# zhanxw/rvtests

Hardware: AMD Instinct MI355X
Metric: gene-sets/sec (SKAT+SKAT-O+CMC+Zeggini, analytic p-values) (higher is better)
Workload: dtype f64

## Files before the change

rvtests_amd/csrc/suffstat_hc.hip.h:

```cpp
#pragma once
#include <type_traits>
#include "suffstat_kernels.hip.h"

namespace rvt {

typedef int i4_t __attribute__((ext_vector_type(4)));
typedef unsigned int u4_t __attribute__((ext_vector_type(4)));

constexpr int kHcMaxMT = 6;
constexpr int kHcMaxD = 13;
constexpr int kHcStepUnit = 12;
constexpr int kHcMaxSteps = 1020;
constexpr int kHcColstatRows = 6;

constexpr int hc_pq_tiles(int MT) { return MT * MT + MT * (MT + 1) / 2; }
constexpr int hc_pq_words(int MT) { return hc_pq_tiles(MT) * 128; }
constexpr int hc_lds_words(int MT) { return hc_pq_words(MT) + 64 * MT + 4; }

struct NullTile {
  const double* base;
  int cols;
};

__device__ __forceinline__ unsigned row16_sum(unsigned h) {
  h += (unsigned)__builtin_amdgcn_update_dpp(0, (int)h, 0xB1, 0xF, 0xF, true);
  h += (unsigned)__builtin_amdgcn_update_dpp(0, (int)h, 0x4E, 0xF, 0xF, true);
  h += (unsigned)__builtin_amdgcn_update_dpp(0, (int)h, 0x141, 0xF, 0xF, true);
  h += (unsigned)__builtin_amdgcn_update_dpp(0, (int)h, 0x140, 0xF, 0xF, true);
  return h;
}

template <int MT>
struct HcStep {
  u4_t glo[MT], ghi[MT];
  u4_t xlo, xhi;
};

template <int MT, bool NT>
__device__ __forceinline__ void hc_issue(HcStep<MT>& f, const __amdgpu_buffer_rsrc_t& rg, const unsigned (&voff)[MT],
                                         const __amdgpu_buffer_rsrc_t& rx, unsigned xoff, int imm) {
#pragma unroll
  for (int c = 0; c < MT; ++c) {
    f.glo[c] = __builtin_bit_cast(u4_t, __builtin_amdgcn_raw_buffer_load_b128(rg, voff[c] + imm, 0, NT ? 2 : 0));
    f.ghi[c] = __builtin_bit_cast(u4_t, __builtin_amdgcn_raw_buffer_load_b128(rg, voff[c] + imm + 16, 0, NT ? 2 : 0));
  }
  f.xlo = __builtin_bit_cast(u4_t, __builtin_amdgcn_raw_buffer_load_b128(rx, xoff + imm, 0, 0));
  f.xhi = __builtin_bit_cast(u4_t, __builtin_amdgcn_raw_buffer_load_b128(rx, xoff + imm + 16, 0, 0));
}

__device__ __forceinline__ double hc_dbl(unsigned lo, unsigned hi) {
  return __builtin_bit_cast(double, ((unsigned long long)hi << 32) | lo);
}

struct HcBurden {
  double a_cmc, a_zeg;
  unsigned zz, cnt;
};

template <bool MASKED>
__device__ __forceinline__ void hc_row(const u4_t& glo, const u4_t& ghi, const double (&xv)[4], d4_t& accT,
                                       unsigned& pk, unsigned& mk, unsigned& cs, unsigned fx, unsigned& h, bool valid) {
  const double g0 = hc_dbl(glo[0], glo[1]), g1 = hc_dbl(glo[2], glo[3]), g2 = hc_dbl(ghi[0], ghi[1]),
               g3 = hc_dbl(ghi[2], ghi[3]);
  accT = __builtin_amdgcn_mfma_f64_16x16x4f64(g0, xv[0], accT, 0, 0, 0);
  accT = __builtin_amdgcn_mfma_f64_16x16x4f64(g1, xv[1], accT, 0, 0, 0);
  accT = __builtin_amdgcn_mfma_f64_16x16x4f64(g2, xv[2], accT, 0, 0, 0);
  accT = __builtin_amdgcn_mfma_f64_16x16x4f64(g3, xv[3], accT, 0, 0, 0);
  const unsigned w01 = __builtin_amdgcn_perm(glo[3], glo[1], 0x0c0c0703u);
  const unsigned w23 = __builtin_amdgcn_perm(ghi[3], ghi[1], 0x07030c0cu);
  unsigned p = ((w01 | w23) >> 5) & 0x03030303u;
  constexpr unsigned kAdd = 0x00100000u, kBits = 0xBFEFFFFFu;
  const unsigned i0 = ((glo[1] + kAdd) & kBits) | glo[0], i1 = ((glo[3] + kAdd) & kBits) | glo[2],
                 i2 = ((ghi[1] + kAdd) & kBits) | ghi[0], i3 = ((ghi[3] + kAdd) & kBits) | ghi[2];
  auto one = [](unsigned x) { return x < 1u ? x : 1u; };
  unsigned m = one(i0) | (one(i1) << 8) | (one(i2) << 16) | (one(i3) << 24);
  if (MASKED) {
    p = valid ? p : 0u;
    m = valid ? m : 0u;
  }
  const unsigned m3 = m * 3u;
  p &= ~m3;
  pk = p;
  mk = m;
  cs = __builtin_amdgcn_sad_u8(p, 0u, cs);
  const unsigned t = (p ^ fx) & ~m3;
  h += (t | (t >> 1)) & 0x01010101u;
}
__device__ __forceinline__ unsigned hc_code3(unsigned p) { return p & (p >> 1) & 0x01010101u; }

__device__ __forceinline__ void hc_note_masked(const u4_t& glo, const u4_t& ghi, unsigned mk, unsigned* oa) {
  auto note = [&](unsigned lo, unsigned hi) {
    __hip_atomic_fetch_or(oa + 0, lo, __ATOMIC_RELAXED, __HIP_MEMORY_SCOPE_WORKGROUP);
    __hip_atomic_fetch_or(oa + 1, hi, __ATOMIC_RELAXED, __HIP_MEMORY_SCOPE_WORKGROUP);
    __hip_atomic_fetch_and(oa + 2, lo, __ATOMIC_RELAXED, __HIP_MEMORY_SCOPE_WORKGROUP);
    __hip_atomic_fetch_and(oa + 3, hi, __ATOMIC_RELAXED, __HIP_MEMORY_SCOPE_WORKGROUP);
  };
  if (mk & 0x000000ffu) note(glo[0], glo[1]);
  if (mk & 0x0000ff00u) note(glo[2], glo[3]);
  if (mk & 0x00ff0000u) note(ghi[0], ghi[1]);
  if (mk & 0xff000000u) note(ghi[2], ghi[3]);
}

template <bool MASKED>
__device__ __forceinline__ void hc_finish(unsigned h, const double (&xv)[4], HcBurden& bu, unsigned vmask) {
  h = row16_sum(h);
  if (MASKED) h &= vmask;
#pragma unroll
  for (int l = 0; l < 4; ++l) {
    const unsigned cz = (h >> (8 * l)) & 0xffu;
    const unsigned cc = cz ? 1u : 0u;
    bu.zz = cz * cz + bu.zz;
    bu.cnt += cc;
    bu.a_zeg = fma((double)cz, xv[l], bu.a_zeg);
    bu.a_cmc = fma((double)cc, xv[l], bu.a_cmc);
  }
}

struct HcMaskCtx {
  unsigned* oa;
  unsigned* flag;
};

template <int MT, bool MASKED>
__device__ __forceinline__ void hc_step(const HcStep<MT>& f, const int T, d4_t (&accT)[MT], unsigned (&pk)[MT][4],
                                        unsigned (&cs)[MT], const unsigned (&fx)[MT], HcBurden& bu, bool valid,
                                        unsigned vmask, unsigned& anym, const HcMaskCtx& mc) {
  double xv[4] = {hc_dbl(f.xlo[0], f.xlo[1]), hc_dbl(f.xlo[2], f.xlo[3]), hc_dbl(f.xhi[0], f.xhi[1]),
                  hc_dbl(f.xhi[2], f.xhi[3])};
  if (MASKED) {
#pragma unroll
    for (int l = 0; l < 4; ++l) xv[l] = valid ? xv[l] : 0.0;
  }
  unsigned h = 0;
#pragma unroll
  for (int c = 0; c < MT; ++c) {
    unsigned p, m;
    hc_row<MASKED>(f.glo[c], f.ghi[c], xv, accT[c], p, m, cs[c], fx[c], h, valid);
    if (m) hc_note_masked(f.glo[c], f.ghi[c], m, mc.oa + 64 * c);
    if (hc_code3(p)) __hip_atomic_fetch_or(mc.flag, 2u, __ATOMIC_RELAXED, __HIP_MEMORY_SCOPE_WORKGROUP);
    pk[c][T] = p | (m << 2);
    anym |= m;
  }
  hc_finish<MASKED>(h, xv, bu, vmask);
}

template <int MT>
__device__ __forceinline__ void hc_gram(const unsigned (&pk)[MT][4], i4_t (&accS)[MT * (MT + 1) / 2]) {
  i4_t op[MT];
#pragma unroll
  for (int c = 0; c < MT; ++c) op[c] = i4_t{(int)pk[c][0], (int)pk[c][1], (int)pk[c][2], (int)pk[c][3]};
  int t = 0;
#pragma unroll
  for (int r = 0; r < MT; ++r)
#pragma unroll
    for (int c = r; c < MT; ++c, ++t) accS[t] = __builtin_amdgcn_mfma_i32_16x16x64_i8(op[r], op[c], accS[t], 0, 0, 0);
}

template <int MT>
__device__ __forceinline__ void hc_gram_masked(const unsigned (&pk)[MT][4], unsigned* lds, int lane) {
  auto mask_op = [&](int c) {
    return i4_t{(int)((pk[c][0] >> 2) & 0x01010101u), (int)((pk[c][1] >> 2) & 0x01010101u),
                (int)((pk[c][2] >> 2) & 0x01010101u), (int)((pk[c][3] >> 2) & 0x01010101u)};
  };
  auto add = [&](int tile, const i4_t& z) {
    const unsigned w0 = (unsigned)z[0] | ((unsigned)z[1] << 16), w1 = (unsigned)z[2] | ((unsigned)z[3] << 16);
    __hip_atomic_fetch_add(lds + (tile * 2 + 0) * 64 + lane, w0, __ATOMIC_RELAXED, __HIP_MEMORY_SCOPE_WORKGROUP);
    __hip_atomic_fetch_add(lds + (tile * 2 + 1) * 64 + lane, w1, __ATOMIC_RELAXED, __HIP_MEMORY_SCOPE_WORKGROUP);
  };
#pragma unroll
  for (int c = 0; c < MT; ++c) {
    const i4_t mc = mask_op(c);
#pragma unroll
    for (int r = 0; r < MT; ++r) {
      const i4_t a = i4_t{(int)pk[r][0], (int)pk[r][1], (int)pk[r][2], (int)pk[r][3]};
      add(r * MT + c, __builtin_amdgcn_mfma_i32_16x16x64_i8(a, mc, i4_t{0, 0, 0, 0}, 0, 0, 0));
      if (r <= c) {
        const i4_t mr = (r == c) ? mc : mask_op(r);
        add(MT * MT + r * MT - r * (r - 1) / 2 + (c - r), __builtin_amdgcn_mfma_i32_16x16x64_i8(mr, mc, i4_t{0, 0, 0, 0}, 0, 0, 0));
      }
    }
    __builtin_amdgcn_sched_barrier(0);
  }
  __hip_atomic_fetch_or(lds + hc_pq_words(MT) + 64 * MT, 1u, __ATOMIC_RELAXED, __HIP_MEMORY_SCOPE_WORKGROUP);
}

template <int MT>
__device__ __forceinline__ void hc_group_end(const unsigned (&pk)[MT][4], i4_t (&accS)[MT * (MT + 1) / 2], unsigned& anym,
                                             unsigned* lds, int lane) {
  hc_gram<MT>(pk, accS);
  if (__builtin_amdgcn_ballot_w64(anym != 0u) != 0ull) hc_gram_masked<MT>(pk, lds, lane);
  anym = 0u;
}

template <int MT, int DEPTH, bool NT>
__device__ __forceinline__ void suffstat_hc_body(const GeneDesc& gd, const NullTile& nt, long long N, long long ld,
                                                 int d, unsigned* lds) {
  const int lane = threadIdx.x & 63;
  const int v = lane & 15, q = lane >> 4;
  const int wpart = blockIdx.x;
  if (wpart >= gd.n_wparts) return;
  constexpr int kPQ = hc_pq_words(MT);
#pragma unroll 4
  for (int w = lane; w < kPQ; w += 64) lds[w] = 0u;
#pragma unroll
  for (int c = 0; c < MT; ++c) lds[kPQ + 64 * c + lane] = (lane & 2) ? 0xffffffffu : 0u;
  if (lane < 4) lds[kPQ + 64 * MT + lane] = 0u;
  const HcMaskCtx mc{lds + kPQ + 4 * v, lds + kPQ + 64 * MT};
  unsigned anym = 0u;
  const long long nsteps = ld >> 4;
  const long long s_begin = (long long)wpart * gd.steps_per_wpart;
  long long s_end = s_begin + gd.steps_per_wpart;
  if (s_end > nsteps) s_end = nsteps;
  if (s_begin >= s_end) return;
  const int M = gd.M;
  auto uniform = [](const void* p) {
    const unsigned long long a = (unsigned long long)p;
    const unsigned lo = __builtin_amdgcn_readfirstlane((unsigned)a);
    const unsigned hi = __builtin_amdgcn_readfirstlane((unsigned)(a >> 32));
    return (void*)(((unsigned long long)hi << 32) | lo);
  };
  const unsigned gbytes = (unsigned)((unsigned long long)M * (unsigned long long)ld * 8ull);
  const __amdgpu_buffer_rsrc_t rg = __builtin_amdgcn_make_buffer_rsrc(uniform(gd.G), 0, gbytes, 0x00020000);
  const unsigned xbytes = (unsigned)((unsigned long long)(d + 1) * (unsigned long long)ld * 8ull);
  const __amdgpu_buffer_rsrc_t rx = __builtin_amdgcn_make_buffer_rsrc(uniform(nt.base), 0, xbytes, 0x00020000);
  const unsigned lane_off = (unsigned)(q * 32);
  const unsigned col_bytes = (unsigned)((unsigned long long)ld * 8ull);
  unsigned vbase[MT];
#pragma unroll
  for (int c = 0; c < MT; ++c) {
    const int col = c * 16 + v;
    vbase[c] = (col < M) ? (unsigned)col * col_bytes + lane_off : 0x80000000u;
  }
  const unsigned xbase = (v <= d) ? (unsigned)v * col_bytes + lane_off : 0x80000000u;
  unsigned fx[MT];
#pragma unroll
  for (int c = 0; c < MT; ++c) fx[c] = ((gd.pflip[c] >> v) & 1) ? 0x02020202u : 0u;

  d4_t accT[MT];
  i4_t accS[MT * (MT + 1) / 2];
  unsigned cs[MT], pk[MT][4];
#pragma unroll
  for (int c = 0; c < MT; ++c) {
    accT[c] = d4_t{0.0, 0.0, 0.0, 0.0};
    cs[c] = 0;
  }
#pragma unroll
  for (int t = 0; t < MT * (MT + 1) / 2; ++t) accS[t] = i4_t{0, 0, 0, 0};
  HcBurden bu{0.0, 0.0, 0u, 0u};

  long long s = s_begin;
  const long long full = N >> 4;
  const long long s_fast_end = (s_end < full) ? s_end : full;
  constexpr int U = (DEPTH == 3) ? 12 : 4;
  const long long n_fast = (s_fast_end > s_begin) ? (s_fast_end - s_begin) / U : 0;
  if constexpr (DEPTH == 1) {
   if (n_fast > 0) {
    unsigned voff[MT];
#pragma unroll
    for (int c = 0; c < MT; ++c) voff[c] = vbase[c] + (unsigned)(s_begin * 128);
    unsigned xoff = xbase + (unsigned)(s_begin * 128);
    u4_t glo[MT], ghi[MT], xlo[2], xhi[2];
#pragma unroll
    for (int c = 0; c < MT; ++c) {
      glo[c] = __builtin_bit_cast(u4_t, __builtin_amdgcn_raw_buffer_load_b128(rg, voff[c], 0, NT ? 2 : 0));
      ghi[c] = __builtin_bit_cast(u4_t, __builtin_amdgcn_raw_buffer_load_b128(rg, voff[c] + 16, 0, NT ? 2 : 0));
    }
    xlo[0] = __builtin_bit_cast(u4_t, __builtin_amdgcn_raw_buffer_load_b128(rx, xoff, 0, 0));
    xhi[0] = __builtin_bit_cast(u4_t, __builtin_amdgcn_raw_buffer_load_b128(rx, xoff + 16, 0, 0));
    for (long long it = 0; it < n_fast; ++it) {
#pragma unroll
      for (int u = 0; u < 4; ++u) {
        xlo[(u + 1) & 1] = __builtin_bit_cast(u4_t, __builtin_amdgcn_raw_buffer_load_b128(rx, xoff + (u + 1) * 128, 0, 0));
        xhi[(u + 1) & 1] = __builtin_bit_cast(u4_t, __builtin_amdgcn_raw_buffer_load_b128(rx, xoff + (u + 1) * 128 + 16, 0, 0));
        __builtin_amdgcn_sched_barrier(0);
        const double xv[4] = {hc_dbl(xlo[u & 1][0], xlo[u & 1][1]), hc_dbl(xlo[u & 1][2], xlo[u & 1][3]),
                              hc_dbl(xhi[u & 1][0], xhi[u & 1][1]), hc_dbl(xhi[u & 1][2], xhi[u & 1][3])};
        unsigned h = 0;
#pragma unroll
        for (int c = 0; c < MT; ++c) {
          unsigned p, m;
          hc_row<false>(glo[c], ghi[c], xv, accT[c], p, m, cs[c], fx[c], h, true);
          if (m) hc_note_masked(glo[c], ghi[c], m, mc.oa + 64 * c);
          if (hc_code3(p)) __hip_atomic_fetch_or(mc.flag, 2u, __ATOMIC_RELAXED, __HIP_MEMORY_SCOPE_WORKGROUP);
          pk[c][u] = p | (m << 2);
          anym |= m;
          glo[c] = __builtin_bit_cast(u4_t, __builtin_amdgcn_raw_buffer_load_b128(rg, voff[c] + (u + 1) * 128, 0, NT ? 2 : 0));
          ghi[c] = __builtin_bit_cast(u4_t, __builtin_amdgcn_raw_buffer_load_b128(rg, voff[c] + (u + 1) * 128 + 16, 0, NT ? 2 : 0));
          __builtin_amdgcn_sched_barrier(0);
        }
        hc_finish<false>(h, xv, bu, 0xffffffffu);
        if (u == 3) hc_group_end<MT>(pk, accS, anym, lds, lane);
        __builtin_amdgcn_sched_barrier(0);
      }
#pragma unroll
      for (int c = 0; c < MT; ++c) voff[c] += 4 * 128;
      xoff += 4 * 128;
    }
    s += n_fast * U;
   }
  } else if (n_fast > 0) {
    unsigned voff[MT];
#pragma unroll
    for (int c = 0; c < MT; ++c) voff[c] = vbase[c] + (unsigned)(s_begin * 128);
    unsigned xoff = xbase + (unsigned)(s_begin * 128);
    HcStep<MT> f[DEPTH];
#pragma unroll
    for (int u = 0; u < DEPTH - 1; ++u) hc_issue<MT, NT>(f[u], rg, voff, rx, xoff, u * 128);
    for (long long it = 0; it < n_fast; ++it) {
#pragma unroll
      for (int u = 0; u < U; ++u) {
        hc_issue<MT, NT>(f[(u + DEPTH - 1) % DEPTH], rg, voff, rx, xoff, (u + DEPTH - 1) * 128);
        __builtin_amdgcn_sched_barrier(0);
        hc_step<MT, false>(f[u % DEPTH], u & 3, accT, pk, cs, fx, bu, true, 0xffffffffu, anym, mc);
        if ((u & 3) == 3) hc_group_end<MT>(pk, accS, anym, lds, lane);
        __builtin_amdgcn_sched_barrier(0);
      }
#pragma unroll
      for (int c = 0; c < MT; ++c) voff[c] += U * 128;
      xoff += U * 128;
    }
    s += n_fast * U;
  }
  while (s < s_end) {
#pragma unroll
    for (int c = 0; c < MT; ++c) pk[c][0] = pk[c][1] = pk[c][2] = pk[c][3] = 0u;
    auto one = [&](const int T, long long su) {
      const bool valid = su < s_end;
      const long long sc = valid ? su : s_end - 1;
      unsigned voff[MT];
#pragma unroll
      for (int c = 0; c < MT; ++c) voff[c] = vbase[c] + (unsigned)(sc * 128);
      HcStep<MT> f;
      hc_issue<MT, false>(f, rg, voff, rx, xbase + (unsigned)(sc * 128), 0);
      unsigned vmask = 0u;
      const long long smp = sc * 16 + q * 4;
#pragma unroll
      for (int l = 0; l < 4; ++l) vmask |= (valid && smp + l < N) ? (0xffu << (8 * l)) : 0u;
      hc_step<MT, true>(f, T, accT, pk, cs, fx, bu, valid, vmask, anym, mc);
    };
    one(0, s);
    one(1, s + 1);
    one(2, s + 2);
    one(3, s + 3);
    hc_group_end<MT>(pk, accS, anym, lds, lane);
    s += 4;
  }

  double* out = gd.parts + (long long)wpart * gd.Mp * gd.Cp;
  const int Cp = gd.Cp;
  {
    int t = 0;
#pragma unroll
    for (int r = 0; r < MT; ++r)
#pragma unroll
      for (int c = r; c < MT; ++c, ++t) {
        const int col = c * 16 + v;
        if (col < M) {
#pragma unroll
          for (int i = 0; i < 4; ++i) out[(long long)(r * 16 + q * 4 + i) * Cp + col] = (double)accS[t][i];
        }
      }
  }
#pragma unroll
  for (int r = 0; r < MT; ++r) {
#pragma unroll
    for (int i = 0; i < 4; ++i) {
      const int row = r * 16 + q + 4 * i;
      if (M + v < Cp) out[(long long)row * Cp + M + v] = accT[r][i];
      if (M + 16 + v < Cp) out[(long long)row * Cp + M + 16 + v] = 0.0;
    }
  }
  long long cnt_w = ((s_end * 16 < N) ? s_end * 16 : N) - s_begin * 16;
  if (cnt_w < 0) cnt_w = 0;
  double* cst = gd.colstat + (long long)wpart * kHcColstatRows * gd.Mp;
  const unsigned wflag = lds[kPQ + 64 * MT];
  {
    int t = 0;
#pragma unroll
    for (int c = 0; c < MT; ++c) {
      unsigned sc = cs[c];
      sc += __shfl_xor(sc, 16, 64);
      sc += __shfl_xor(sc, 32, 64);
      const i4_t dg = accS[t];
      const int sel = (lane & 3) == 0 ? dg[0] : ((lane & 3) == 1 ? dg[1] : ((lane & 3) == 2 ? dg[2] : dg[3]));
      const int diag = __shfl(sel, v + 16 * (v >> 2), 64);
      const int tq = MT * MT + t;
      const unsigned qw = lds[(tq * 2 + ((v >> 1) & 1)) * 64 + v + 16 * (v >> 2)];
      const long long nm = (long long)((qw >> (16 * (v & 1))) & 0xffffu);
      t += MT - c;
      const long long sm = (long long)sc, hh = (long long)diag - 16 * nm, n2 = (hh - sm) / 2, n1 = 2 * sm - hh,
                      n0 = cnt_w - n1 - n2 - nm;
      const double mn = n0 > 0 ? 0.0 : (n1 > 0 ? 1.0 : (n2 > 0 ? 2.0 : INFINITY));
      const double mx = n2 > 0 ? 2.0 : (n1 > 0 ? 1.0 : (n0 > 0 ? 0.0 : -INFINITY));
      if (lane < 16) {
        const int j = c * 16 + lane;
        cst[j] = (double)sm;
        cst[gd.Mp + j] = mn;
        cst[2 * gd.Mp + j] = mx;
        cst[3 * gd.Mp + j] = (double)nm;
        const unsigned* w = lds + kPQ + 64 * c + 4 * lane;
        unsigned long long* bits = reinterpret_cast<unsigned long long*>(cst);
        bits[4 * gd.Mp + j] = ((unsigned long long)w[1] << 32) | w[0];
        bits[5 * gd.Mp + j] = ((unsigned long long)w[3] << 32) | w[2];
      }
    }
  }
  if (gd.wflags && lane == 0) gd.wflags[wpart] = wflag;
  if ((wflag & 1u) && gd.pq) {
    unsigned* dst = gd.pq + (long long)wpart * kPQ;
#pragma unroll 4
    for (int w = lane; w < kPQ; w += 64) dst[w] = lds[w];
  }
  if (gd.bparts) {
    double ac = bu.a_cmc, az = bu.a_zeg;
    ac += __shfl_xor(ac, 16, 64);
    az += __shfl_xor(az, 16, 64);
    ac += __shfl_xor(ac, 32, 64);
    az += __shfl_xor(az, 32, 64);
    unsigned zz = bu.zz, cn = bu.cnt;
    zz += __shfl_xor(zz, 16, 64);
    cn += __shfl_xor(cn, 16, 64);
    zz += __shfl_xor(zz, 32, 64);
    cn += __shfl_xor(cn, 32, 64);
    const int rl = 3 + d;
    double* bp = gd.bparts + (long long)wpart * 2 * rl;
    if (lane <= d) {
      const int k = (lane == d) ? 0 : 3 + lane;
      bp[k] = ac;
      bp[rl + k] = az;
    }
    if (lane == 0) {
      bp[1] = (double)cn;
      bp[2] = (double)cn;
      bp[rl + 1] = (double)zz;
      bp[rl + 2] = (double)cn;
    }
  }
}

template <int MT, int DEPTH, int WAVES, bool NT>
__global__ __launch_bounds__(64, WAVES) void gene_suffstat_hc(const GeneDesc* __restrict__ genes, NullTile nt,
                                                              long long N, long long ld, int d) {
  __shared__ unsigned lds[hc_lds_words(MT)];
  const GeneDesc gd = genes[blockIdx.y];
  if (gd.MT != MT) return;
  suffstat_hc_body<MT, DEPTH, NT>(gd, nt, N, ld, d, lds);
}

#define RVT_HC_ONE_WAVE __launch_bounds__(64) __attribute__((amdgpu_waves_per_eu(1, 1)))
template <int MT, int DEPTH, bool NT>
__global__ RVT_HC_ONE_WAVE void gene_suffstat_hc_one(const GeneDesc* __restrict__ genes, NullTile nt, long long N,
                                                     long long ld, int d) {
  __shared__ unsigned lds[hc_lds_words(MT)];
  const GeneDesc gd = genes[blockIdx.y];
  if (gd.MT != MT) return;
  suffstat_hc_body<MT, DEPTH, NT>(gd, nt, N, ld, d, lds);
}

constexpr int kHcAnyMaxMT = 5;
constexpr int hc_any_depth(int MT) { return MT == 2 ? 4 : (MT == 3 ? 3 : (MT == 4 ? 2 : (MT == 5 ? 1 : 0))); }
template <bool NT>
__global__ RVT_HC_ONE_WAVE void gene_suffstat_hc_any(const GeneDesc* __restrict__ genes, NullTile nt, long long N,
                                                              long long ld, int d, unsigned classes) {
  __shared__ unsigned lds[hc_lds_words(kHcAnyMaxMT)];
  const GeneDesc gd = genes[blockIdx.y];
  if (!((classes >> gd.MT) & 1u)) return;
  switch (gd.MT) {
    case 2: suffstat_hc_body<2, hc_any_depth(2), NT>(gd, nt, N, ld, d, lds); break;
    case 3: suffstat_hc_body<3, hc_any_depth(3), NT>(gd, nt, N, ld, d, lds); break;
    case 4: suffstat_hc_body<4, hc_any_depth(4), NT>(gd, nt, N, ld, d, lds); break;
    case 5: suffstat_hc_body<5, hc_any_depth(5), NT>(gd, nt, N, ld, d, lds); break;
    default: break;
  }
}

template <int UNUSED = 0>
__global__ __launch_bounds__(256) void block_classify_kernel(const double* __restrict__ G, long long N, long long ld,
                                                             int M, int* __restrict__ flag) {
  const long long per_col = (N + 1) / 2;
  const long long total = per_col * M;
  bool bad = false;
  for (long long idx = blockIdx.x * (long long)blockDim.x + threadIdx.x; idx < total;
       idx += (long long)gridDim.x * blockDim.x) {
    const long long j = idx / per_col, i = (idx % per_col) * 2;
    const unsigned long long* p = reinterpret_cast<const unsigned long long*>(G + j * ld + i);
    const unsigned long long a = p[0], b = (i + 1 < N) ? p[1] : 0ull;
    auto ok = [](unsigned long long x) {
      return x == 0ull || x == 0x3FF0000000000000ull || x == 0x4000000000000000ull;
    };
    bad |= !ok(a) || !ok(b);
  }
  if (__any(bad) && (threadIdx.x & 63) == 0) atomicAnd(flag, 0);
}

}
```

Before: 26730.

## Batch masked-genotype side effects per step and keep MT=4 masked Gram in registers

In the one-wave kernels, the per-column masked-note and code-3 atomic side effects are moved out of the inner column loop. They are now gated by a single wave-wide ballot per step, which drops per-column divergent branches on the hot path. For MT=4 with depth 2, the masked P/Q Gram partials are kept in packed 16-bit VGPR accumulators instead of LDS atomics and are written to LDS once at the end. Per-column any-mask tracking also lets it skip MFMAs for columns with no masked entries. The costs are higher register pressure and a packed 16-bit accumulator that could overflow if a wave sees very many masked entries.

New measurement: 27030, median of 2. No clear change (+1.1%).

```diff
diff --git a/rvtests_amd/csrc/suffstat_hc.hip.h b/rvtests_amd/csrc/suffstat_hc.hip.h
--- a/rvtests_amd/csrc/suffstat_hc.hip.h
+++ b/rvtests_amd/csrc/suffstat_hc.hip.h
@@ -121,25 +121,44 @@
   unsigned* flag;
 };
 
-template <int MT, bool MASKED>
+template <int MT, bool PQR>
+struct HcPq {
+  unsigned r[PQR ? hc_pq_tiles(MT) : 1][2];
+  unsigned any[PQR ? MT : 1];
+};
+
+template <int MT, bool MASKED, bool LONE, bool PQR>
 __device__ __forceinline__ void hc_step(const HcStep<MT>& f, const int T, d4_t (&accT)[MT], unsigned (&pk)[MT][4],
                                         unsigned (&cs)[MT], const unsigned (&fx)[MT], HcBurden& bu, bool valid,
-                                        unsigned vmask, unsigned& anym, const HcMaskCtx& mc) {
+                                        unsigned vmask, unsigned& anym, const HcMaskCtx& mc, HcPq<MT, PQR>& pq) {
   double xv[4] = {hc_dbl(f.xlo[0], f.xlo[1]), hc_dbl(f.xlo[2], f.xlo[3]), hc_dbl(f.xhi[0], f.xhi[1]),
                   hc_dbl(f.xhi[2], f.xhi[3])};
   if (MASKED) {
 #pragma unroll
     for (int l = 0; l < 4; ++l) xv[l] = valid ? xv[l] : 0.0;
   }
-  unsigned h = 0;
+  unsigned h = 0, ms[MT], mstep = 0u, c3 = 0u;
 #pragma unroll
   for (int c = 0; c < MT; ++c) {
-    unsigned p, m;
-    hc_row<MASKED>(f.glo[c], f.ghi[c], xv, accT[c], p, m, cs[c], fx[c], h, valid);
-    if (m) hc_note_masked(f.glo[c], f.ghi[c], m, mc.oa + 64 * c);
-    if (hc_code3(p)) __hip_atomic_fetch_or(mc.flag, 2u, __ATOMIC_RELAXED, __HIP_MEMORY_SCOPE_WORKGROUP);
-    pk[c][T] = p | (m << 2);
-    anym |= m;
+    unsigned p;
+    hc_row<MASKED>(f.glo[c], f.ghi[c], xv, accT[c], p, ms[c], cs[c], fx[c], h, valid);
+    if constexpr (!LONE) {
+      if (ms[c]) hc_note_masked(f.glo[c], f.ghi[c], ms[c], mc.oa + 64 * c);
+      if (hc_code3(p)) __hip_atomic_fetch_or(mc.flag, 2u, __ATOMIC_RELAXED, __HIP_MEMORY_SCOPE_WORKGROUP);
+    }
+    c3 |= hc_code3(p);
+    pk[c][T] = p | (ms[c] << 2);
+    mstep |= ms[c];
+    if constexpr (PQR) pq.any[c] |= ms[c];
+  }
+  anym |= mstep;
+  if constexpr (LONE) {
+    if (__builtin_expect(__builtin_amdgcn_ballot_w64((mstep | c3) != 0u) != 0ull, 0)) {
+#pragma unroll
+      for (int c = 0; c < MT; ++c)
+        if (ms[c]) hc_note_masked(f.glo[c], f.ghi[c], ms[c], mc.oa + 64 * c);
+      if (c3) __hip_atomic_fetch_or(mc.flag, 2u, __ATOMIC_RELAXED, __HIP_MEMORY_SCOPE_WORKGROUP);
+    }
   }
   hc_finish<MASKED>(h, xv, bu, vmask);
 }
@@ -184,15 +203,63 @@
   __hip_atomic_fetch_or(lds + hc_pq_words(MT) + 64 * MT, 1u, __ATOMIC_RELAXED, __HIP_MEMORY_SCOPE_WORKGROUP);
 }
 
+constexpr bool hc_pq_in_regs(int MT, int DEPTH) { return MT == 4 && DEPTH == 2; }
+template <int MT>
+__device__ __forceinline__ void hc_gram_masked_regs(const unsigned (&pk)[MT][4], unsigned (&pqr)[hc_pq_tiles(MT)][2],
+                                                    unsigned (&any)[MT], unsigned* flag) {
+  auto mask_op = [&](int c) {
+    return i4_t{(int)((pk[c][0] >> 2) & 0x01010101u), (int)((pk[c][1] >> 2) & 0x01010101u),
+                (int)((pk[c][2] >> 2) & 0x01010101u), (int)((pk[c][3] >> 2) & 0x01010101u)};
+  };
+  auto row_op = [&](int r) { return i4_t{(int)pk[r][0], (int)pk[r][1], (int)pk[r][2], (int)pk[r][3]}; };
+  auto add = [&](const int tile, const i4_t& z) {
+    unsigned &w0 = pqr[tile][0], &w1 = pqr[tile][1];
+    w0 += (unsigned)z[0] | ((unsigned)z[1] << 16);
+    w1 += (unsigned)z[2] | ((unsigned)z[3] << 16);
+    asm volatile("" : "+v"(w0), "+v"(w1));
+  };
+#pragma unroll
+  for (int c = 0; c < MT; ++c) {
+    if (__builtin_amdgcn_ballot_w64(any[c] != 0u) != 0ull) {
+      const i4_t mc = mask_op(c);
+      i4_t zp[MT], zq[MT];
+#pragma unroll
+      for (int r = 0; r < MT; ++r) zp[r] = __builtin_amdgcn_mfma_i32_16x16x64_i8(row_op(r), mc, i4_t{0, 0, 0, 0}, 0, 0, 0);
+#pragma unroll
+      for (int r = 0; r <= c; ++r)
+        zq[r] = __builtin_amdgcn_mfma_i32_16x16x64_i8((r == c) ? mc : mask_op(r), mc, i4_t{0, 0, 0, 0}, 0, 0, 0);
+      __builtin_amdgcn_sched_barrier(0);
+#pragma unroll
+      for (int r = 0; r < MT; ++r) add(r * MT + c, zp[r]);
+#pragma unroll
+      for (int r = 0; r <= c; ++r) add(MT * MT + r * MT - r * (r - 1) / 2 + (c - r), zq[r]);
+    }
+    any[c] = 0u;
+    __builtin_amdgcn_sched_barrier(0);
+  }
+  __hip_atomic_fetch_or(flag, 1u, __ATOMIC_RELAXED, __HIP_MEMORY_SCOPE_WORKGROUP);
+}
+
+template <int MT, bool PQR>
+__device__ __forceinline__ void hc_group_end(const unsigned (&pk)[MT][4], i4_t (&accS)[MT * (MT + 1) / 2], unsigned& anym,
+                                             unsigned* lds, int lane, HcPq<MT, PQR>& pq) {
+  hc_gram<MT>(pk, accS);
+  if (__builtin_amdgcn_ballot_w64(anym != 0u) != 0ull) {
+    if constexpr (PQR)
+      hc_gram_masked_regs<MT>(pk, pq.r, pq.any, lds + hc_pq_words(MT) + 64 * MT);
+    else
+      hc_gram_masked<MT>(pk, lds, lane);
+  }
+  anym = 0u;
+}
 template <int MT>
 __device__ __forceinline__ void hc_group_end(const unsigned (&pk)[MT][4], i4_t (&accS)[MT * (MT + 1) / 2], unsigned& anym,
                                              unsigned* lds, int lane) {
-  hc_gram<MT>(pk, accS);
-  if (__builtin_amdgcn_ballot_w64(anym != 0u) != 0ull) hc_gram_masked<MT>(pk, lds, lane);
-  anym = 0u;
-}
-
-template <int MT, int DEPTH, bool NT>
+  HcPq<MT, false> none;
+  hc_group_end<MT, false>(pk, accS, anym, lds, lane, none);
+}
+
+template <int MT, int DEPTH, bool NT, bool LONE = false, bool PQR = false>
 __device__ __forceinline__ void suffstat_hc_body(const GeneDesc& gd, const NullTile& nt, long long N, long long ld,
                                                  int d, unsigned* lds) {
   const int lane = threadIdx.x & 63;
@@ -247,6 +314,13 @@
 #pragma unroll
   for (int t = 0; t < MT * (MT + 1) / 2; ++t) accS[t] = i4_t{0, 0, 0, 0};
   HcBurden bu{0.0, 0.0, 0u, 0u};
+  HcPq<MT, PQR> pq;
+  if constexpr (PQR) {
+#pragma unroll
+    for (int t = 0; t < hc_pq_tiles(MT); ++t) pq.r[t][0] = pq.r[t][1] = 0u;
+#pragma unroll
+    for (int c = 0; c < MT; ++c) pq.any[c] = 0u;
+  }
 
   long long s = s_begin;
   const long long full = N >> 4;
@@ -289,7 +363,7 @@
           __builtin_amdgcn_sched_barrier(0);
         }
         hc_finish<false>(h, xv, bu, 0xffffffffu);
-        if (u == 3) hc_group_end<MT>(pk, accS, anym, lds, lane);
+        if (u == 3) hc_group_end<MT, PQR>(pk, accS, anym, lds, lane, pq);
         __builtin_amdgcn_sched_barrier(0);
       }
 #pragma unroll
@@ -311,8 +385,8 @@
       for (int u = 0; u < U; ++u) {
         hc_issue<MT, NT>(f[(u + DEPTH - 1) % DEPTH], rg, voff, rx, xoff, (u + DEPTH - 1) * 128);
         __builtin_amdgcn_sched_barrier(0);
-        hc_step<MT, false>(f[u % DEPTH], u & 3, accT, pk, cs, fx, bu, true, 0xffffffffu, anym, mc);
-        if ((u & 3) == 3) hc_group_end<MT>(pk, accS, anym, lds, lane);
+        hc_step<MT, false, LONE, PQR>(f[u % DEPTH], u & 3, accT, pk, cs, fx, bu, true, 0xffffffffu, anym, mc, pq);
+        if ((u & 3) == 3) hc_group_end<MT, PQR>(pk, accS, anym, lds, lane, pq);
         __builtin_amdgcn_sched_barrier(0);
       }
 #pragma unroll
@@ -336,16 +410,23 @@
       const long long smp = sc * 16 + q * 4;
 #pragma unroll
       for (int l = 0; l < 4; ++l) vmask |= (valid && smp + l < N) ? (0xffu << (8 * l)) : 0u;
-      hc_step<MT, true>(f, T, accT, pk, cs, fx, bu, valid, vmask, anym, mc);
+      hc_step<MT, true, LONE, PQR>(f, T, accT, pk, cs, fx, bu, valid, vmask, anym, mc, pq);
     };
     one(0, s);
     one(1, s + 1);
     one(2, s + 2);
     one(3, s + 3);
-    hc_group_end<MT>(pk, accS, anym, lds, lane);
+    hc_group_end<MT, PQR>(pk, accS, anym, lds, lane, pq);
     s += 4;
   }
 
+  if constexpr (PQR) {
+#pragma unroll
+    for (int t = 0; t < hc_pq_tiles(MT); ++t) {
+      lds[(t * 2 + 0) * 64 + lane] = pq.r[t][0];
+      lds[(t * 2 + 1) * 64 + lane] = pq.r[t][1];
+    }
+  }
   double* out = gd.parts + (long long)wpart * gd.Mp * gd.Cp;
   const int Cp = gd.Cp;
   {
@@ -454,7 +535,7 @@
   __shared__ unsigned lds[hc_lds_words(MT)];
   const GeneDesc gd = genes[blockIdx.y];
   if (gd.MT != MT) return;
-  suffstat_hc_body<MT, DEPTH, NT>(gd, nt, N, ld, d, lds);
+  suffstat_hc_body<MT, DEPTH, NT, true, hc_pq_in_regs(MT, DEPTH)>(gd, nt, N, ld, d, lds);
 }
 
 constexpr int kHcAnyMaxMT = 5;
@@ -466,10 +547,10 @@
   const GeneDesc gd = genes[blockIdx.y];
   if (!((classes >> gd.MT) & 1u)) return;
   switch (gd.MT) {
-    case 2: suffstat_hc_body<2, hc_any_depth(2), NT>(gd, nt, N, ld, d, lds); break;
-    case 3: suffstat_hc_body<3, hc_any_depth(3), NT>(gd, nt, N, ld, d, lds); break;
-    case 4: suffstat_hc_body<4, hc_any_depth(4), NT>(gd, nt, N, ld, d, lds); break;
-    case 5: suffstat_hc_body<5, hc_any_depth(5), NT>(gd, nt, N, ld, d, lds); break;
+    case 2: suffstat_hc_body<2, hc_any_depth(2), NT, true>(gd, nt, N, ld, d, lds); break;
+    case 3: suffstat_hc_body<3, hc_any_depth(3), NT, true>(gd, nt, N, ld, d, lds); break;
+    case 4: suffstat_hc_body<4, hc_any_depth(4), NT, true, hc_pq_in_regs(4, hc_any_depth(4))>(gd, nt, N, ld, d, lds); break;
+    case 5: suffstat_hc_body<5, hc_any_depth(5), NT, true>(gd, nt, N, ld, d, lds); break;
     default: break;
   }
 }
```
